# castorini/dhr

Measured on AMD Instinct MI355X. Metric: queries/sec (exact top-1000, brute-force dense-hybrid GIP retrieval), higher is better.
Workload: dtype i8 (bound GEMM: gated AND ungated columns int8 x int8 -> int32 on the matrix cores, every gated rounding upward, the ungated quantisation error paid by the filter margin) + f64-accumulated f16 x f32 exact rescoring of the survivors -- the returned scores are the exact scores rounded once, identical

## Files before the change

### dhr_amd/csrc/kernels.hip

```cpp
#include <algorithm>
#include <cstdlib>
#include <mutex>

#include "dhr_internal.h"
#include "gemm_common.h"
#include <type_traits>

namespace dhr {

typedef short short8 __attribute__((ext_vector_type(8)));

static hipError_t ensure_lds_attr(const void* fn, int bytes, int (&have)[64]) {
  static std::mutex mu;
  int dev = 0;
  (void)hipGetDevice(&dev);
  std::lock_guard<std::mutex> lock(mu);
  if (bytes <= have[dev & 63]) return hipSuccess;
  const hipError_t e = hipFuncSetAttribute(fn, hipFuncAttributeMaxDynamicSharedMemorySize, bytes);
  if (e == hipSuccess) have[dev & 63] = bytes;
  return e;
}

__device__ __forceinline__ float wave_sum(float v) {
#pragma unroll
// ... 1117 lines not shown
#pragma unroll
      for (int u = 0; u < U; ++u) {
        if constexpr (PB == 8) { const uint2 t = gather8(r + u * 128); v[u].w[0] = t.x; v[u].w[1] = t.y; }
        else { const uint4 t = gather16(r + u * 128); v[u].w[0] = t.x; v[u].w[1] = t.y; v[u].w[WPP - 2] = t.z; v[u].w[WPP - 1] = t.w; }
      }
    }
  };
  uint2 c;
  Piece v[U];
  fetch(base + (threadIdx.x / LPC), c, v);
  for (uint32_t i = base + (threadIdx.x / LPC); i < base + REFINE_PER_WG; i += CPR) {
    uint2 cn;
    Piece vn[U];
    fetch(i + CPR < base + REFINE_PER_WG ? i + CPR : 0xffffffffu, cn, vn);
    int isum = 0;
#pragma unroll
    for (int u = 0; u < U; ++u) {
#pragma unroll
      for (int h = 0; h < WPP; ++h) {
        isum = __builtin_amdgcn_sdot4((int)fe[WPP * u + h], (int)(v[u].w[h] & 0x0f0f0f0fu), isum, false);
        isum = __builtin_amdgcn_sdot4((int)fo[WPP * u + h], (int)((v[u].w[h] >> 4) & 0x0f0f0f0fu), isum, false);
      }
    }
#pragma unroll
    for (int o = 1; o < LPC; o <<= 1) isum += __shfl_xor(isum, o, 64);
    if (sub == 0 && i < count) {
      float u2 = __uint_as_float(c.y) + sa * (float)(isum - off);
      u2 += fabsf(u2) * 4.8e-7f;
      if (u2 >= t) {
        const uint32_t slot = atomicAdd(p.out_cnt + q, 1u);
        if (slot < p.out_cap) p.out[(int64_t)q * p.out_cap + slot] = make_uint2(c.x, __float_as_uint(u2));
      }
    }
    c = cn;
#pragma unroll
    for (int u = 0; u < U; ++u) v[u] = vn[u];
  }
  if (!p.blk_off) return;
  }
}
hipError_t launch_refine(const RefineArgs& a, hipStream_t s) {
  if (a.max_count == 0 || a.n_queries <= 0) return hipSuccess;
  if (a.resid8) {
    const dim3 grid = a.blk_off ? dim3(std::min<uint32_t>(a.flat_blocks, FLAT_GRID_MAX)) : dim3((a.max_count + REFINE_PER_WG - 1) / REFINE_PER_WG, (unsigned)a.n_queries);
    if (a.blk_off && !a.flat_blocks) return hipSuccess;
    switch (a.resid_ld / 8) {
      case 16: hipLaunchKernelGGL(dense_refine_kernel<16>, grid, dim3(256), 0, s, a); break;
      case 32: hipLaunchKernelGGL(dense_refine_kernel<32>, grid, dim3(256), 0, s, a); break;
      case 48: hipLaunchKernelGGL(dense_refine_kernel<48>, grid, dim3(256), 0, s, a); break;
      case 64: hipLaunchKernelGGL(dense_refine_kernel<64>, grid, dim3(256), 0, s, a); break;
      default: return hipErrorInvalidValue;
    }
    return hipGetLastError();
  }
  const bool g8 = a.g8_q8 != nullptr;
  const size_t lds = (size_t)a.d_dlr * (g8 ? 8 : 4);
  const dim3 grid = a.blk_off ? dim3(std::min<uint32_t>(a.flat_blocks, FLAT_GRID_MAX)) : dim3((a.max_count + REFINE_PER_WG - 1) / REFINE_PER_WG, (unsigned)a.n_queries);
  if (a.blk_off && !a.flat_blocks) return hipSuccess;
  if (g8) hipLaunchKernelGGL(refine_kernel<true>, grid, dim3(256), lds, s, a);
  else hipLaunchKernelGGL(refine_kernel<false>, grid, dim3(256), lds, s, a);
  return hipGetLastError();
}

__device__ __forceinline__ float fmix_lo(uint32_t a, uint32_t b) { float r; asm("v_fma_mix_f32 %0, %1, %2, 0 op_sel_hi:[1,1,0]" : "=v"(r) : "v"(a), "v"(b)); return r; }
__device__ __forceinline__ float fmix_hi(uint32_t a, uint32_t b) { float r; asm("v_fma_mix_f32 %0, %1, %2, 0 op_sel:[1,1,0] op_sel_hi:[1,1,0]" : "=v"(r) : "v"(a), "v"(b)); return r; }
typedef unsigned short ushort2v __attribute__((ext_vector_type(2)));
__device__ __forceinline__ uint32_t pair_mask(uint32_t x, uint32_t sel) {
  union { uint32_t u; ushort2v v; } t, one;
  t.u = __builtin_amdgcn_perm(0u, x, sel);
  one.u = 0x00010001u;
  t.v = __builtin_elementwise_min(t.v, one.v);
  t.v = t.v - one.v;
  return t.u;
}
__device__ __forceinline__ uint32_t pair_mask16(uint32_t x) {
  union { uint32_t u; ushort2v v; } t, one;
  t.u = x;
  one.u = 0x00010001u;
  t.v = __builtin_elementwise_min(t.v, one.v);
  t.v = t.v - one.v;
  return t.u;
}
template <int PATH>
__device__ __forceinline__ void rescore_block(const RescoreArgs& p, const int q, const uint32_t blk) {
  const int lane = threadIdx.x & 63;
  const int wave = threadIdx.x >> 6;
  uint32_t count;
  if (p.cand) { count = p.cnt[q]; if (count > p.cap) count = p.cap; }
  else if (p.rows32) count = p.count_all;
  else count = p.count_all;
  const uint32_t base = blk * RESCORE_CANDS_PER_WG;
  if (base >= count) return;
  const float* q32 = p.q32 + (int64_t)q * p.k_rm;
  const int16_t* qi = p.q_idx + (int64_t)q * p.d_dlr;
  const int nchunks = p.k_rm >> 3;
  const int dlr_chunks = p.d_dlr >> 3;
  const bool fast = p.q16 && *p.q_inexact == 0u && (!p.gate || p.d_dlr == 0 || p.c_idx_dtype == DHR_IDX_U8 || p.c_idx_dtype == DHR_IDX_I8);
  const bool some_zero = p.q_inexact && p.q_inexact[1] != 0u;
  uint32_t nz_mask = some_zero ? 0u : 0xFFFFFFFFu;
  for (int c = lane, t = 0; some_zero && c < nchunks; c += 64, ++t) {
    const float4 qa = *(const float4*)(q32 + c * 8);
    const float4 qb = *(const float4*)(q32 + c * 8 + 4);
    if (qa.x != 0.f || qa.y != 0.f || qa.z != 0.f || qa.w != 0.f || qb.x != 0.f || qb.y != 0.f || qb.z != 0.f || qb.w != 0.f) nz_mask |= 1u << t;
  }
  if constexpr (PATH == 0) {
    if (p.split && p.q16 && *p.q_inexact == 0u && some_zero) {
      int m = 0;
      for (int t = 0; t * 64 < nchunks; ++t) m += __popcll(__ballot((nz_mask >> t) & 1u));
      if (m <= 16) return;
    }
  }
  if constexpr (PATH == 3) {
    if (!(p.q16 && *p.q_inexact == 0u && some_zero)) return;
    const bool idx16 = p.c_idx_dtype == DHR_IDX_I16;
    int nzc[16];
    int m = 0;
    for (int c0 = 0, t = 0; c0 < nchunks && m <= 16; c0 += 64, ++t) {
      uint64_t b = __ballot((nz_mask >> t) & 1u);
      while (b && m <= 16) { if (m < 16) nzc[m] = c0 + (__ffsll((unsigned long long)b) - 1); ++m; b &= b - 1; }
    }
    if (m > 16) return;
    {
      auto run = [&](auto lanes_c) __attribute__((always_inline)) {
        constexpr int L = decltype(lanes_c)::value, P = 64 / L;
        const int ci = lane / L, sl = lane % L;
        int myc = -1;
#pragma unroll
        for (int e = 0; e < L; ++e) if (e < m && sl == e) myc = nzc[e];
        uint4 qv = make_uint4(0u, 0u, 0u, 0u);
        uint4 qix = make_uint4(0u, 0u, 0u, 0u);
        const bool gated_chunk = myc >= 0 && myc < dlr_chunks && p.gate;
        if (myc >= 0) qv = *(const uint4*)(p.q16 + (int64_t)q * p.k_rm + myc * 8);
        if (gated_chunk) {
          if (idx16) qix = *(const uint4*)(p.q_idx + (int64_t)q * p.d_dlr + myc * 8);
          else { const uint2 t8 = *(const uint2*)(p.q_idx8 + (int64_t)q * p.d_dlr + myc * 8); qix.x = t8.x; qix.y = t8.y; }
        }
        static_assert(RESCORE_CANDS_PER_WG % (4 * P) == 0, "4 waves x P pairs per round");
        for (uint32_t i0 = base + wave * P; i0 < base + RESCORE_CANDS_PER_WG && i0 < count; i0 += 4 * P) {
          const uint32_t i = i0 + ci;
          const bool live = i < count;
          uint32_t row = 0u;
          if (live) {
            if (p.cand) row = p.cand[(int64_t)q * p.cap + i].x;
            else if (p.rows32) row = p.rows32[(int64_t)q * p.ld_rows + i];
            else row = (uint32_t)(p.row0 + i);
          }
          const bool valid = live && (int64_t)row < p.n_rows;
          double acc = 0.0;
          if (valid && myc >= 0) {
            const uint4 dv = *(const uint4*)(p.vals_rm + (int64_t)row * p.k_rm + myc * 8);
            uint32_t d[4] = {dv.x, dv.y, dv.z, dv.w};
            const uint32_t qq[4] = {qv.x, qv.y, qv.z, qv.w};
            if (gated_chunk && idx16) {
              const uint4 cix = *(const uint4*)((const int16_t*)p.c_idx + (int64_t)row * p.d_dlr + myc * 8);
              d[0] &= pair_mask16(cix.x ^ qix.x); d[1] &= pair_mask16(cix.y ^ qix.y);
              d[2] &= pair_mask16(cix.z ^ qix.z); d[3] &= pair_mask16(cix.w ^ qix.w);
            } else if (gated_chunk) {
              const uint2 cix = *(const uint2*)((const uint8_t*)p.c_idx + (int64_t)row * p.d_dlr + myc * 8);
              const uint32_t x0 = cix.x ^ qix.x, x1 = cix.y ^ qix.y;
              d[0] &= pair_mask(x0, 0x0c010c00u); d[1] &= pair_mask(x0, 0x0c030c02u);
              d[2] &= pair_mask(x1, 0x0c010c00u); d[3] &= pair_mask(x1, 0x0c030c02u);
            }
#pragma unroll
            for (int e = 0; e < 4; ++e) {
              acc += (double)fmix_lo(d[e], qq[e]);
              acc += (double)fmix_hi(d[e], qq[e]);
            }
          }
#pragma unroll
          for (int o = 1; o < L; o <<= 1) acc += __shfl_xor(acc, o, 64);
          if (sl == 0 && live) {
            const float sc = valid ? (float)acc : -INFINITY;
            if (p.out_keys) p.out_keys[(int64_t)q * p.ld_keys + i] = valid ? make_key(sc, row) : 0ull;
            if (p.out_scores && q < p.n_queries) p.out_scores[(int64_t)q * p.ld_scores + i] = sc;
          }
        }
      };
      if (m <= 8) run(std::integral_constant<int, 8>{}); else run(std::integral_constant<int, 16>{});
      return;
    }
  }
  if constexpr (PATH != 3) {
  if constexpr (PATH == 0 || PATH == 2)
  if (fast && !some_zero && nchunks <= 128) {
#ifndef RESCORE_NARROW_L
#define RESCORE_NARROW_L 16
#endif
    constexpr int L = RESCORE_NARROW_L, P = 64 / L;
    const int g = lane / L, sl = lane % L;
    static_assert(RESCORE_CANDS_PER_WG % (4 * P) == 0, "4 waves x P pairs per round");
    for (uint32_t i0 = base + wave * P; i0 < base + RESCORE_CANDS_PER_WG && i0 < count; i0 += 4 * P) {
      const uint32_t i = i0 + g;
      const bool live = i < count;
      uint32_t row = 0u;
      if (live) {
        if (p.cand) row = p.cand[(int64_t)q * p.cap + i].x;
        else if (p.rows32) row = p.rows32[(int64_t)q * p.ld_rows + i];
        else row = (uint32_t)(p.row0 + i);
      }
      const bool valid = live && (int64_t)row < p.n_rows;
      double acc = 0.0;
      if (valid) {
        for (int c = sl; c < nchunks; c += L) {
          const uint4 dv = gather16(p.vals_rm + (int64_t)row * p.k_rm + c * 8);
          const uint4 qv = *(const uint4*)(p.q16 + (int64_t)q * p.k_rm + c * 8);
          uint32_t d[4] = {dv.x, dv.y, dv.z, dv.w};
          const uint32_t qq[4] = {qv.x, qv.y, qv.z, qv.w};
          if (c < dlr_chunks && p.gate) {
            const uint2 ci = gather8((const uint8_t*)p.c_idx + (int64_t)row * p.d_dlr + c * 8);
            const uint2 qi8 = *(const uint2*)(p.q_idx8 + (int64_t)q * p.d_dlr + c * 8);
            const uint32_t x0 = ci.x ^ qi8.x, x1 = ci.y ^ qi8.y;
            d[0] &= pair_mask(x0, 0x0c010c00u); d[1] &= pair_mask(x0, 0x0c030c02u);
            d[2] &= pair_mask(x1, 0x0c010c00u); d[3] &= pair_mask(x1, 0x0c030c02u);
          }
#pragma unroll
          for (int e = 0; e < 4; ++e) {
            acc += (double)fmix_lo(d[e], qq[e]);
            acc += (double)fmix_hi(d[e], qq[e]);
          }
        }
      }
#pragma unroll
      for (int o = L / 2; o > 0; o >>= 1) acc += __shfl_xor(acc, o, 64);
      if (sl == 0 && live) {
        const float sc = valid ? (float)acc : -INFINITY;
        if (p.out_keys) p.out_keys[(int64_t)q * p.ld_keys + i] = valid ? make_key(sc, row) : 0ull;
        if (p.out_scores && q < p.n_queries) p.out_scores[(int64_t)q * p.ld_scores + i] = sc;
      }
    }
    return;
  }
  if constexpr (PATH != 2)
  for (uint32_t i = base + wave; i < base + RESCORE_CANDS_PER_WG && i < count; i += 4) {
    uint32_t row;
    if (p.cand) row = p.cand[(int64_t)q * p.cap + i].x;
    else if (p.rows32) row = p.rows32[(int64_t)q * p.ld_rows + i];
    else row = (uint32_t)(p.row0 + i);
    const bool valid = (int64_t)row < p.n_rows;
    double acc = 0.0;
    if (valid && fast) {
      for (int c = lane; c < nchunks; c += 64) {
        if (!((nz_mask >> (c >> 6)) & 1u)) continue;
        const uint4 dv = gather16(p.vals_rm + (int64_t)row * p.k_rm + c * 8);
        const uint4 qv = *(const uint4*)(p.q16 + (int64_t)q * p.k_rm + c * 8);
        uint32_t d[4] = {dv.x, dv.y, dv.z, dv.w};
        const uint32_t qq[4] = {qv.x, qv.y, qv.z, qv.w};
        if (c < dlr_chunks && p.gate) {
          const uint2 ci = gather8((const uint8_t*)p.c_idx + (int64_t)row * p.d_dlr + c * 8);
          const uint2 qi8 = *(const uint2*)(p.q_idx8 + (int64_t)q * p.d_dlr + c * 8);
          const uint32_t x0 = ci.x ^ qi8.x, x1 = ci.y ^ qi8.y;
          d[0] &= pair_mask(x0, 0x0c010c00u); d[1] &= pair_mask(x0, 0x0c030c02u);
          d[2] &= pair_mask(x1, 0x0c010c00u); d[3] &= pair_mask(x1, 0x0c030c02u);
        }
#pragma unroll
        for (int e = 0; e < 4; ++e) {
          acc += (double)fmix_lo(d[e], qq[e]);
          acc += (double)fmix_hi(d[e], qq[e]);
        }
      }
      acc = wave_sum_f64(acc);
    } else if (PATH == 0 && valid) {
      for (int c = lane; c < nchunks; c += 64) {
        if (!((nz_mask >> (c >> 6)) & 1u)) continue;
        const half8 dv = *(const half8*)(p.vals_rm + (int64_t)row * p.k_rm + c * 8);
        const float4 qa = *(const float4*)(q32 + c * 8);
        const float4 qb = *(const float4*)(q32 + c * 8 + 4);
        const float qv[8] = {qa.x, qa.y, qa.z, qa.w, qb.x, qb.y, qb.z, qb.w};
        if (c < dlr_chunks && p.gate) {
          int ci[8];
          if (p.c_idx_dtype == DHR_IDX_I16) {
            const short8 v = *(const short8*)((const int16_t*)p.c_idx + (int64_t)row * p.d_dlr + c * 8);
#pragma unroll
            for (int e = 0; e < 8; ++e) ci[e] = v[e];
          } else {
            const uint2 v = *(const uint2*)((const uint8_t*)p.c_idx + (int64_t)row * p.d_dlr + c * 8);
#pragma unroll
            for (int e = 0; e < 8; ++e) {
              const uint32_t w = (e < 4) ? v.x : v.y;
              const uint32_t byte = (w >> (8 * (e & 3))) & 0xFFu;
              ci[e] = (p.c_idx_dtype == DHR_IDX_I8) ? (int)(int8_t)byte : (int)byte;
            }
          }
          const short8 qiv = *(const short8*)(qi + c * 8);
#pragma unroll
          for (int e = 0; e < 8; ++e) {
            const double d = (ci[e] == (int)qiv[e]) ? (double)(float)dv[e] : 0.0;
            acc = fma(d, (double)qv[e], acc);
          }
        } else {
#pragma unroll
          for (int e = 0; e < 8; ++e) acc = fma((double)(float)dv[e], (double)qv[e], acc);
        }
      }
      acc = wave_sum_f64(acc);
    }
    if (lane == 0) {
      const float sc = valid ? (float)acc : -INFINITY;
      if (p.out_keys) p.out_keys[(int64_t)q * p.ld_keys + i] = valid ? make_key(sc, row) : 0ull;
      if (p.out_scores && q < p.n_queries) p.out_scores[(int64_t)q * p.ld_scores + i] = sc;
    }
  }
  }
}
#ifndef RESCORE_WPE
#define RESCORE_WPE 7
#endif
__device__ __forceinline__ bool rescore_fast_batch(const RescoreArgs& p) {
  return p.q16 && p.q_inexact[0] == 0u && p.q_inexact[1] == 0u &&
         (!p.gate || p.d_dlr == 0 || p.c_idx_dtype == DHR_IDX_U8 || p.c_idx_dtype == DHR_IDX_I8);
}
template <int PATH>
__device__ __forceinline__ void rescore_run(const RescoreArgs& p) {
  if (!p.blk_off) { rescore_block<PATH>(p, (int)blockIdx.y, blockIdx.x); return; }
  for (uint32_t b = blockIdx.x;; b += gridDim.x) {
    int q; uint32_t blk;
    if (!flat_block(p.blk_off, p.n_queries, b, q, blk)) return;
    rescore_block<PATH>(p, q, blk);
  }
}
__global__ void __launch_bounds__(256) __attribute__((amdgpu_waves_per_eu(RESCORE_WPE))) rescore_kernel(RescoreArgs p) {
  if (p.split && rescore_fast_batch(p)) return;
  rescore_run<0>(p);
}
__global__ void __launch_bounds__(256) __attribute__((amdgpu_waves_per_eu(8))) rescore_fast_kernel(RescoreArgs p) {
  if (!rescore_fast_batch(p) || (p.k_rm >> 3) <= 128) return;
  rescore_run<1>(p);
}
__global__ void __launch_bounds__(256) __attribute__((amdgpu_waves_per_eu(8))) rescore_sparse_kernel(RescoreArgs p) {
  if (!p.q16 || p.q_inexact[0] != 0u || p.q_inexact[1] == 0u) return;
  rescore_run<3>(p);
}
__global__ void __launch_bounds__(256) __attribute__((amdgpu_waves_per_eu(8))) rescore_narrow_kernel(RescoreArgs p) {
  if (!rescore_fast_batch(p) || (p.k_rm >> 3) > 128) return;
  rescore_run<2>(p);
}
hipError_t launch_rescore(const RescoreArgs& a_in, hipStream_t s) {
  if (a_in.max_count == 0 || a_in.n_queries <= 0) return hipSuccess;
  RescoreArgs a = a_in;
  a.split = (a.q16 && a.q_inexact) ? 1 : 0;
  const bool wide = (a.k_rm >> 3) > 128;
  dim3 grid;
  if (a.blk_off) {
    if (!a.flat_blocks) return hipSuccess;
    grid = dim3(std::min<uint32_t>(a.flat_blocks, FLAT_GRID_MAX));
  } else grid = dim3((a.max_count + RESCORE_CANDS_PER_WG - 1) / RESCORE_CANDS_PER_WG, (unsigned)a.n_queries);
  if (a.split && wide) hipLaunchKernelGGL(rescore_fast_kernel, grid, dim3(256), 0, s, a);
  if (a.split && !wide) hipLaunchKernelGGL(rescore_narrow_kernel, grid, dim3(256), 0, s, a);
  if (a.split) hipLaunchKernelGGL(rescore_sparse_kernel, grid, dim3(256), 0, s, a);
  hipLaunchKernelGGL(rescore_kernel, grid, dim3(256), 0, s, a);
  return hipGetLastError();
}

__device__ __forceinline__ void bitonic_desc(uint64_t* keys, int n, int tid, int nthreads) {
  for (int size = 2; size <= n; size <<= 1) {
    for (int stride = size >> 1; stride > 0; stride >>= 1) {
      for (int t = tid; t < (n >> 1); t += nthreads) {
        const int pos = 2 * t - (t & (stride - 1));
        const uint64_t a = keys[pos], b = keys[pos + stride];
        const bool desc = (pos & size) == 0;
        if ((a < b) == desc) { keys[pos] = b; keys[pos + stride] = a; }
      }
      __syncthreads();
    }
  }
}

__device__ __forceinline__ int count_greater(const uint64_t* arr, int n, uint64_t key) {
  int lo = 0, hi = n;
  while (lo < hi) {
    const int mid = (lo + hi) >> 1;
    if (arr[mid] > key) lo = mid + 1; else hi = mid;
  }
  return lo;
}

constexpr int SELECT_SM_THREADS = 256;
template <int EA>
__global__ void __launch_bounds__(SELECT_SM_THREADS) select_kernel(SelectArgs p) {
  extern __shared__ __attribute__((aligned(16))) char smem[];
  uint64_t* A = (uint64_t*)smem;
  int& fill = *(int*)(smem + (size_t)p.sort_n * 8);
  const int kps = p.kps;
  uint64_t* B = A + kps;
  const int q = blockIdx.x;
  const int tid = threadIdx.x;
  uint32_t count = p.cnt ? p.cnt[q] : p.count_all;
  if (p.cnt && count > p.cap) count = p.cap;
  uint64_t* topk = p.topk_keys + (int64_t)q * p.kp;
  const uint64_t* in = p.in_keys + (int64_t)q * p.ld_keys;
  for (int j = tid; j < kps; j += SELECT_SM_THREADS) A[j] = topk[j];
  if (tid == 0) fill = 0;
  __syncthreads();
  uint32_t room = 64;
  while (room * 2 <= (uint32_t)(p.sort_n - kps) && room < 2048) room <<= 1;
  const int k_keep = p.k_keep ? p.k_keep : p.k;
  for (uint32_t base = 0; base < count; base += room) {
    const uint64_t kth = A[k_keep - 1];
    __syncthreads();
    const uint32_t end = (base + room < count) ? base + room : count;
    for (uint32_t j = base + tid; j < end; j += SELECT_SM_THREADS) {
      const uint64_t key = in[j];
      if (key > kth) B[atomicAdd(&fill, 1)] = key;
    }
    __syncthreads();
    const int m = fill;
    if (m > 0) {
      int m2 = 2;
      while (m2 < m) m2 <<= 1;
      for (int j = m + tid; j < m2; j += SELECT_SM_THREADS) B[j] = 0ull;
      __syncthreads();
      bitonic_desc(B, m2, tid, SELECT_SM_THREADS);
      uint64_t ka[EA], kb[8];
      int da[EA], db[8];
#pragma unroll
      for (int e = 0; e < EA; ++e) {
        const int i = tid + e * SELECT_SM_THREADS;
        da[e] = kps;
        if (i < kps) { ka[e] = A[i]; da[e] = ka[e] ? i + count_greater(B, m, ka[e]) : kps; }
      }
#pragma unroll
      for (int e = 0; e < 8; ++e) {
        const int j = tid + e * SELECT_SM_THREADS;
        db[e] = kps;
        if (j < m) { kb[e] = B[j]; db[e] = j + count_greater(A, kps, kb[e]); }
      }
      const int total = min(kps, m + count_greater(A, kps, 0ull));
      __syncthreads();
      for (int j = total + tid; j < kps; j += SELECT_SM_THREADS) A[j] = 0ull;
#pragma unroll
      for (int e = 0; e < EA; ++e)
        if (da[e] < kps) A[da[e]] = ka[e];
#pragma unroll
      for (int e = 0; e < 8; ++e)
        if (db[e] < kps) A[db[e]] = kb[e];
    }
    __syncthreads();
    if (tid == 0) fill = 0;
    __syncthreads();
  }
  for (int j = tid; j < kps; j += SELECT_SM_THREADS) topk[j] = (j < k_keep) ? A[j] : 0ull;
  if (tid == 0) {
    const uint64_t kth = A[p.k - 1];
    float t = kth ? ordered_f32((uint32_t)(kth >> 32)) : -INFINITY;
    if (p.monotone) t = fmaxf(t, p.tau[q]);
    p.tau[q] = t;
    p.thr[q] = (q < p.n_queries) ? t - p.margin[q] : INFINITY;
  }
}

constexpr int SELECT_BIG_BATCH = 2048;
constexpr int SELECT_BIG_THREADS = 256;
constexpr int SELECT_BIG_EPT = 4;
__global__ void __launch_bounds__(SELECT_BIG_THREADS) select_big_kernel(SelectArgs p) {
  __shared__ uint64_t B[SELECT_BIG_BATCH];
  __shared__ int fill;
  const int q = blockIdx.x, tid = threadIdx.x;
  uint32_t count = p.cnt ? p.cnt[q] : p.count_all;
  if (p.cnt && count > p.cap) count = p.cap;
  uint64_t* topk = p.topk_keys + (int64_t)q * p.kp;
  const uint64_t* in = p.in_keys + (int64_t)q * p.ld_keys;
  const int k_keep = p.k_keep ? p.k_keep : p.k;
  constexpr int TILE = SELECT_BIG_THREADS * SELECT_BIG_EPT;
  for (uint32_t base = 0; base < count; base += SELECT_BIG_BATCH) {
    if (tid == 0) fill = 0;
    __syncthreads();
    const uint64_t kth = topk[k_keep - 1];
    const uint32_t end = (base + SELECT_BIG_BATCH < count) ? base + SELECT_BIG_BATCH : count;
    for (uint32_t j = base + tid; j < end; j += SELECT_BIG_THREADS) {
      const uint64_t key = in[j];
      if (key > kth) B[atomicAdd(&fill, 1)] = key;
    }
    __syncthreads();
    const int m = fill;
    if (m == 0) continue;
    int m2 = 2;
    while (m2 < m) m2 <<= 1;
    for (int j = m + tid; j < m2; j += SELECT_BIG_THREADS) B[j] = 0ull;
    __syncthreads();
    bitonic_desc(B, m2, tid, SELECT_BIG_THREADS);
    uint64_t kb[SELECT_BIG_BATCH / SELECT_BIG_THREADS]; int db[SELECT_BIG_BATCH / SELECT_BIG_THREADS];
#pragma unroll
    for (int e = 0; e < SELECT_BIG_BATCH / SELECT_BIG_THREADS; ++e) {
      const int j = tid + e * SELECT_BIG_THREADS;
      kb[e] = (j < m) ? B[j] : 0ull;
      db[e] = (j < m) ? j + count_greater(topk, k_keep, kb[e]) : k_keep;
    }
    __syncthreads();
    for (int t0 = (k_keep - 1) / TILE * TILE; t0 >= 0; t0 -= TILE) {
      uint64_t ka[SELECT_BIG_EPT]; int da[SELECT_BIG_EPT];
#pragma unroll
      for (int e = 0; e < SELECT_BIG_EPT; ++e) {
        const int i = t0 + tid + e * SELECT_BIG_THREADS;
        da[e] = k_keep;
        if (i < k_keep) { ka[e] = topk[i]; da[e] = i + count_greater(B, m, ka[e]); }
      }
      __syncthreads();
#pragma unroll
      for (int e = 0; e < SELECT_BIG_EPT; ++e)
        if (da[e] < k_keep) topk[da[e]] = ka[e];
    }
#pragma unroll
    for (int e = 0; e < SELECT_BIG_BATCH / SELECT_BIG_THREADS; ++e)
      if (db[e] < k_keep) topk[db[e]] = kb[e];
  }
  __syncthreads();
  if (tid == 0) {
    const uint64_t kth = topk[p.k - 1];
    float t = kth ? ordered_f32((uint32_t)(kth >> 32)) : -INFINITY;
    if (p.monotone) t = fmaxf(t, p.tau[q]);
    p.tau[q] = t;
    p.thr[q] = (q < p.n_queries) ? t - p.margin[q] : INFINITY;
  }
}

hipError_t launch_select(const SelectArgs& a, hipStream_t s) {
  if (a.kp > 16384) return launch_select_global(a, s);
  if (a.kp > 4096) {
    hipLaunchKernelGGL(select_big_kernel, dim3((unsigned)a.n_queries), dim3(SELECT_BIG_THREADS), 0, s, a);
    return hipGetLastError();
  }
  static int attr_bytes[64] = {}, attr_bytes4[64] = {};
  const int bytes = a.sort_n * 8 + 16;
  if (a.kp <= 4 * SELECT_SM_THREADS) {
    if (hipError_t e = ensure_lds_attr((const void*)select_kernel<4>, bytes, attr_bytes4); e != hipSuccess) return e;
    hipLaunchKernelGGL(select_kernel<4>, dim3((unsigned)a.n_queries), dim3(SELECT_SM_THREADS), bytes, s, a);
    return hipGetLastError();
  }
  if (hipError_t e = ensure_lds_attr((const void*)select_kernel<16>, bytes, attr_bytes); e != hipSuccess) return e;
  hipLaunchKernelGGL(select_kernel<16>, dim3((unsigned)a.n_queries), dim3(SELECT_SM_THREADS), bytes, s, a);
  return hipGetLastError();
}

constexpr int PQ_K = 256;
constexpr int PQ_MAX_DSUB = 64;

template <int DSUB>
__global__ void __launch_bounds__(256) pq_assign_kernel(const __half* __restrict__ vals, int64_t ld, int64_t n, int64_t stride, int dsub_rt,
                                                        const float* __restrict__ cb , uint8_t* __restrict__ codes,
                                                        int64_t ld_codes, float* __restrict__ sums ,
                                                        uint32_t* __restrict__ counts , float* __restrict__ err ,
                                                        int ksub ) {
  __shared__ float c[PQ_K * PQ_MAX_DSUB];
  __shared__ float cn[PQ_K];
  const int dsub = DSUB ? DSUB : dsub_rt;
  const int m = blockIdx.y;
  const float* cbm = cb + (int64_t)m * ksub * dsub;
  for (int i = threadIdx.x; i < ksub * dsub; i += 256) c[i] = cbm[i];
  __syncthreads();
  if ((int)threadIdx.x < ksub) {
    float s = 0.f;
    for (int j = 0; j < dsub; ++j) s += c[threadIdx.x * dsub + j] * c[threadIdx.x * dsub + j];
    cn[threadIdx.x] = s;
  }
  __syncthreads();
  const int64_t pi = (int64_t)blockIdx.x * 256 + threadIdx.x;
  if (pi >= n) return;
  const __half* x = vals + pi * stride * ld + (int64_t)m * dsub;
  float xv[DSUB ? DSUB : PQ_MAX_DSUB];
#pragma unroll
  for (int j = 0; j < (DSUB ? DSUB : PQ_MAX_DSUB); ++j)
    if (j < dsub) xv[j] = __half2float(x[j]);
  float best = INFINITY;
  int arg = 0;
  for (int k = 0; k < ksub; ++k) {
    float dot = 0.f;
#pragma unroll
    for (int j = 0; j < (DSUB ? DSUB : 1); ++j)
      if (DSUB) dot += xv[j] * c[k * dsub + j];
    if (!DSUB)
      for (int j = 0; j < dsub; ++j) dot += xv[j] * c[k * dsub + j];
    const float dist = cn[k] - 2.f * dot;
    if (dist < best) { best = dist; arg = k; }
  }
  if (codes) codes[pi * ld_codes + m] = (uint8_t)arg;
  if (sums) {
    for (int j = 0; j < dsub; ++j) atomicAdd(&sums[((int64_t)m * ksub + arg) * dsub + j], xv[j]);
    atomicAdd(&counts[m * ksub + arg], 1u);
    if (err) {
      float xx = 0.f;
      for (int j = 0; j < dsub; ++j) xx += xv[j] * xv[j];
      atomicAdd(&err[m], best + xx);
    }
  }
}
__global__ void __launch_bounds__(256) pq_update_kernel(float* __restrict__ cb, const float* __restrict__ sums, const uint32_t* __restrict__ counts,
                                                        int dsub, int ksub) {
  const int m = blockIdx.x, k = threadIdx.x;
  __shared__ uint32_t cnt[PQ_K];
  __shared__ int big;
  cnt[k] = k < ksub ? counts[m * ksub + k] : 0u;
  __syncthreads();
  if (k == 0) {
    int b = 0;
    for (int i = 1; i < ksub; ++i) if (cnt[i] > cnt[b]) b = i;
    big = b;
  }
  __syncthreads();
  if (k >= ksub) return;
  float* c = cb + ((int64_t)m * ksub + k) * dsub;
  if (cnt[k] > 0) {
    const float inv = 1.f / (float)cnt[k];
    for (int j = 0; j < dsub; ++j) c[j] = sums[((int64_t)m * ksub + k) * dsub + j] * inv;
  } else {
    const float inv = 1.f / (float)(cnt[big] ? cnt[big] : 1u);
    for (int j = 0; j < dsub; ++j) c[j] = sums[((int64_t)m * ksub + big) * dsub + j] * inv * (1.f + ((j + k) & 1 ? 1.f : -1.f) / 1024.f);
  }
}
__global__ void __launch_bounds__(256) pq_init_kernel(const __half* __restrict__ vals, int64_t ld, int64_t n, int64_t stride, int dsub, int M,
                                                      float* __restrict__ cb, int ksub) {
  const int m = blockIdx.x, k = threadIdx.x;
  if (k >= ksub) return;
  const int64_t pi = (n >= ksub) ? (int64_t)k * (n / ksub) : (int64_t)(k % (n > 0 ? n : 1));
  const __half* x = vals + pi * stride * ld + (int64_t)m * dsub;
  for (int j = 0; j < dsub; ++j) cb[((int64_t)m * ksub + k) * dsub + j] = __half2float(x[j]);
}
__global__ void __launch_bounds__(256) pq_decode_kernel(const uint8_t* __restrict__ codes, int64_t ld_codes, int64_t n, int M, int dsub,
                                                        const float* __restrict__ cb, __half* __restrict__ out, int64_t ld_out, int ksub) {
  const int d = M * dsub;
  const int64_t total = n * d;
  for (int64_t g = (int64_t)blockIdx.x * 256 + threadIdx.x; g < total; g += (int64_t)gridDim.x * 256) {
    const int64_t row = g / d;
    const int col = (int)(g - row * d);
    const int m = col / dsub, j = col - m * dsub;
    out[row * ld_out + col] = __float2half(cb[((int64_t)m * ksub + codes[row * ld_codes + m]) * dsub + j]);
  }
}
hipError_t launch_pq_init(const __half* vals, int64_t ld, int64_t n, int64_t stride, int dsub, int M, float* cb, int ksub, hipStream_t s) {
  hipLaunchKernelGGL(pq_init_kernel, dim3(M), dim3(256), 0, s, vals, ld, n, stride, dsub, M, cb, ksub);
  return hipGetLastError();
}
hipError_t launch_pq_assign(const __half* vals, int64_t ld, int64_t n, int64_t stride, int dsub, int M, const float* cb, uint8_t* codes,
                            int64_t ld_codes, float* sums, uint32_t* counts, float* err, int ksub, hipStream_t s) {
  if (n <= 0) return hipSuccess;
  const dim3 grid((unsigned)((n + 255) / 256), M);
#define PQ_GO(D) hipLaunchKernelGGL(pq_assign_kernel<D>, grid, dim3(256), 0, s, vals, ld, n, stride, dsub, cb, codes, ld_codes, sums, counts, err, ksub)
  if (dsub == 12) PQ_GO(12); else if (dsub == 24) PQ_GO(24); else if (dsub == 14) PQ_GO(14); else if (dsub == 16) PQ_GO(16); else PQ_GO(0);
#undef PQ_GO
  return hipGetLastError();
}
hipError_t launch_pq_update(float* cb, const float* sums, const uint32_t* counts, int dsub, int M, int ksub, hipStream_t s) {
  hipLaunchKernelGGL(pq_update_kernel, dim3(M), dim3(256), 0, s, cb, sums, counts, dsub, ksub);
  return hipGetLastError();
}
hipError_t launch_pq_decode(const uint8_t* codes, int64_t ld_codes, int64_t n, int M, int dsub, const float* cb, __half* out, int64_t ld_out, int ksub,
                            hipStream_t s) {
  if (n <= 0) return hipSuccess;
  const int64_t blocks = std::min<int64_t>((n * M * dsub + 255) / 256, 65536);
  hipLaunchKernelGGL(pq_decode_kernel, dim3((unsigned)blocks), dim3(256), 0, s, codes, ld_codes, n, M, dsub, cb, out, ld_out, ksub);
  return hipGetLastError();
// ... 463 lines not shown
```

Measured before the change: 60370.

## Add templated wide rescore kernel with in-flight row prefetch and register-resident query

Adds a specialised rescore kernel for wide rows, templated on the number of 64-lane chunks (T) and gated index chunks (G). It keeps the query slice in registers, double-buffers candidate row gathers (P rows in flight) so loads overlap the f64 accumulation, and replaces the shuffle reduction with ds_swizzle. Gating masks are computed with packed u16 min/sub. Per-(T,G) waves-per-EU choices are meant to trade occupancy against the register cost of holding several rows in flight, and unsupported shapes fall back to the old kernel.

```diff
diff --git a/dhr_amd/csrc/kernels.hip b/dhr_amd/csrc/kernels.hip
--- a/dhr_amd/csrc/kernels.hip
+++ b/dhr_amd/csrc/kernels.hip
@@ -1443,6 +1443,138 @@
   }
   }
 }
+__device__ __forceinline__ double wave_sum_f64_swz(double v) {
+  v += __shfl_xor(v, 32, 64);
+  auto step = [&](auto o) __attribute__((always_inline)) {
+    constexpr int pat = (decltype(o)::value << 10) | 0x1F;
+    union { double d; int w[2]; } a, b;
+    a.d = v;
+    b.w[0] = __builtin_amdgcn_ds_swizzle(a.w[0], pat);
+    b.w[1] = __builtin_amdgcn_ds_swizzle(a.w[1], pat);
+    v += b.d;
+  };
+  step(std::integral_constant<int, 16>{}); step(std::integral_constant<int, 8>{}); step(std::integral_constant<int, 4>{});
+  step(std::integral_constant<int, 2>{}); step(std::integral_constant<int, 1>{});
+  return v;
+}
+__device__ __forceinline__ uint32_t pair_mask_pk(uint32_t x, uint32_t sel, uint32_t one) {
+  uint32_t t = __builtin_amdgcn_perm(0u, x, sel), r;
+  asm("v_pk_min_u16 %0, %1, %2" : "=v"(r) : "v"(t), "v"(one));
+  asm("v_pk_sub_u16 %0, %1, %2" : "=v"(t) : "v"(r), "v"(one));
+  return t;
+}
+#ifndef RESCORE_WIDE_P
+#define RESCORE_WIDE_P 2
+#endif
+constexpr int rescore_wide_wpe(int T, int G) {
+#ifdef RESCORE_WIDE_WPE
+  return RESCORE_WIDE_WPE;
+#else
+  static_assert(RESCORE_WIDE_P == 2, "the table below was taken from the P = 2 allocation");
+  return T == 3 ? (G <= 2 ? 7 : 6) : (G == 0 ? 7 : G <= 3 ? 5 : 4);
+#endif
+}
+template <int T, int G, int P>
+__device__ __forceinline__ void rescore_block_wide(const RescoreArgs& p, const int q_in, const uint32_t blk_in) {
+  constexpr int NP = RESCORE_CANDS_PER_WG / 4;
+  static_assert(NP <= 64 && G <= T && P >= 1, "one lane per pair of the wave");
+  const int lane = threadIdx.x & 63;
+  const int wave = __builtin_amdgcn_readfirstlane(threadIdx.x >> 6);
+  const int q = __builtin_amdgcn_readfirstlane(q_in);
+  const uint32_t blk = (uint32_t)__builtin_amdgcn_readfirstlane((int)blk_in);
+  uint32_t count;
+  if (p.cand) { count = p.cnt[q]; if (count > p.cap) count = p.cap; }
+  else count = p.count_all;
+  count = (uint32_t)__builtin_amdgcn_readfirstlane((int)count);
+  const uint32_t first = blk * RESCORE_CANDS_PER_WG + wave;
+  if (first >= count) return;
+  const int npairs = (int)min((uint32_t)NP, (count - first + 3u) >> 2);
+  const uint32_t nchunks = (uint32_t)p.k_rm >> 3;
+  const uint32_t dlr_chunks = (uint32_t)p.d_dlr >> 3;
+  const uint32_t i_own = first + 4u * (uint32_t)lane;
+  uint32_t row_own = 0u;
+  bool valid_own = false;
+  if (lane < npairs) {
+    if (p.cand) row_own = p.cand[(int64_t)q * p.cap + i_own].x;
+    else if (p.rows32) row_own = p.rows32[(int64_t)q * p.ld_rows + i_own];
+    else row_own = (uint32_t)(p.row0 + i_own);
+    valid_own = (int64_t)row_own < p.n_rows;
+  }
+  const uint32_t row_ld = valid_own ? row_own : 0u;
+  const uint32_t c_last = (uint32_t)lane + 64u * (T - 1);
+  const bool live_last = c_last < nchunks;
+  const uint32_t voff0 = (uint32_t)lane * 16u, voff_last = (live_last ? c_last : nchunks - 1u) * 16u;
+  const uint32_t g_last = (uint32_t)lane + 64u * (G > 0 ? G - 1 : 0);
+  const bool gated_last = g_last < dlr_chunks;
+  const uint32_t xoff0 = (uint32_t)lane * 8u, xoff_last = (gated_last ? g_last : dlr_chunks - 1u) * 8u;
+  const uint32_t gmask_last = gated_last ? 0xFFFFFFFFu : 0u;
+  uint4 qv[T];
+  uint2 qx[G > 0 ? G : 1];
+  {
+    const char* q16 = (const char*)(p.q16 + (int64_t)q * p.k_rm);
+#pragma unroll
+    for (int t = 0; t < T; ++t) qv[t] = *(const uint4*)(q16 + (t < T - 1 ? voff0 + 1024u * t : voff_last));
+    if constexpr (G > 0) {
+      const char* q8 = (const char*)(p.q_idx8 + (int64_t)q * p.d_dlr);
+#pragma unroll
+      for (int t = 0; t < G; ++t) qx[t] = *(const uint2*)(q8 + (t < G - 1 ? xoff0 + 512u * t : xoff_last));
+    }
+  }
+  uint4 dv[P][T];
+  uint2 dx[P][G > 0 ? G : 1];
+  auto issue = [&](const int s, const uint32_t row) __attribute__((always_inline)) {
+    uint32_t v0 = voff0, v1 = voff_last, x0 = xoff0, x1 = xoff_last;
+    asm volatile("" : "+v"(v0), "+v"(v1), "+v"(x0), "+v"(x1));
+    const char* r = (const char*)(p.vals_rm + (int64_t)row * p.k_rm);
+#pragma unroll
+    for (int t = 0; t < T; ++t) dv[s][t] = gather16(r + (t < T - 1 ? v0 + 1024u * t : v1));
+    if constexpr (G > 0) {
+      const char* x = (const char*)p.c_idx + (int64_t)row * p.d_dlr;
+#pragma unroll
+      for (int t = 0; t < G; ++t) dx[s][t] = gather8(x + (t < G - 1 ? x0 + 512u * t : x1));
+    }
+  };
+  const uint32_t one = 0x00010001u;
+  auto chunk = [&](double acc, const int s, const int t) __attribute__((always_inline)) -> double {
+    uint32_t d[4] = {dv[s][t].x, dv[s][t].y, dv[s][t].z, dv[s][t].w};
+    const uint32_t qq[4] = {qv[t].x, qv[t].y, qv[t].z, qv[t].w};
+    if (t < G) {
+      uint32_t x0 = dx[s][t].x ^ qx[t].x, x1 = dx[s][t].y ^ qx[t].y;
+      if (t == G - 1) { x0 &= gmask_last; x1 &= gmask_last; }
+      d[0] &= pair_mask_pk(x0, 0x0c010c00u, one); d[1] &= pair_mask_pk(x0, 0x0c030c02u, one);
+      d[2] &= pair_mask_pk(x1, 0x0c010c00u, one); d[3] &= pair_mask_pk(x1, 0x0c030c02u, one);
+    }
+#pragma unroll
+    for (int e = 0; e < 4; ++e) {
+      acc += (double)fmix_lo(d[e], qq[e]);
+      acc += (double)fmix_hi(d[e], qq[e]);
+    }
+    return acc;
+  };
+#pragma unroll
+  for (int j = 0; j < P && j < NP; ++j) issue(j, (uint32_t)__builtin_amdgcn_readlane((int)row_ld, j));
+#pragma unroll
+  for (int t = 0; t < T; ++t) asm volatile("" : "+v"(qv[t].x), "+v"(qv[t].y), "+v"(qv[t].z), "+v"(qv[t].w));
+  float res = 0.f;
+#pragma unroll
+  for (int j = 0; j < NP; ++j) {
+    if (j >= npairs) break;
+    const int s = j % P;
+    double acc = 0.0;
+#pragma unroll
+    for (int t = 0; t < T - 1; ++t) acc = chunk(acc, s, t);
+    if (live_last) acc = chunk(acc, s, T - 1);
+    __builtin_amdgcn_sched_barrier(0);
+    if (j + P < NP) issue(s, (uint32_t)__builtin_amdgcn_readlane((int)row_ld, j + P));
+    acc = wave_sum_f64_swz(acc);
+    if (lane == j) res = (float)acc;
+  }
+  if (lane < npairs) {
+    const float sc = valid_own ? res : -INFINITY;
+    if (p.out_keys) p.out_keys[(int64_t)q * p.ld_keys + i_own] = valid_own ? make_key(sc, row_own) : 0ull;
+    if (p.out_scores && q < p.n_queries) p.out_scores[(int64_t)q * p.ld_scores + i_own] = sc;
+  }
+}
 #ifndef RESCORE_WPE
 #define RESCORE_WPE 7
 #endif
@@ -1450,14 +1582,18 @@
   return p.q16 && p.q_inexact[0] == 0u && p.q_inexact[1] == 0u &&
          (!p.gate || p.d_dlr == 0 || p.c_idx_dtype == DHR_IDX_U8 || p.c_idx_dtype == DHR_IDX_I8);
 }
-template <int PATH>
-__device__ __forceinline__ void rescore_run(const RescoreArgs& p) {
-  if (!p.blk_off) { rescore_block<PATH>(p, (int)blockIdx.y, blockIdx.x); return; }
+template <class F>
+__device__ __forceinline__ void rescore_for_blocks(const RescoreArgs& p, F block) {
+  if (!p.blk_off) { block((int)blockIdx.y, blockIdx.x); return; }
   for (uint32_t b = blockIdx.x;; b += gridDim.x) {
     int q; uint32_t blk;
     if (!flat_block(p.blk_off, p.n_queries, b, q, blk)) return;
-    rescore_block<PATH>(p, q, blk);
-  }
+    block(q, blk);
+  }
+}
+template <int PATH>
+__device__ __forceinline__ void rescore_run(const RescoreArgs& p) {
+  rescore_for_blocks(p, [&](const int q, const uint32_t blk) __attribute__((always_inline)) { rescore_block<PATH>(p, q, blk); });
 }
 __global__ void __launch_bounds__(256) __attribute__((amdgpu_waves_per_eu(RESCORE_WPE))) rescore_kernel(RescoreArgs p) {
   if (p.split && rescore_fast_batch(p)) return;
@@ -1466,6 +1602,11 @@
 __global__ void __launch_bounds__(256) __attribute__((amdgpu_waves_per_eu(8))) rescore_fast_kernel(RescoreArgs p) {
   if (!rescore_fast_batch(p) || (p.k_rm >> 3) <= 128) return;
   rescore_run<1>(p);
+}
+template <int T, int G>
+__global__ void __launch_bounds__(256) __attribute__((amdgpu_waves_per_eu(rescore_wide_wpe(T, G)))) rescore_fast_kernel_wide(RescoreArgs p) {
+  if (!rescore_fast_batch(p)) return;
+  rescore_for_blocks(p, [&](const int q, const uint32_t blk) __attribute__((always_inline)) { rescore_block_wide<T, G, RESCORE_WIDE_P>(p, q, blk); });
 }
 __global__ void __launch_bounds__(256) __attribute__((amdgpu_waves_per_eu(8))) rescore_sparse_kernel(RescoreArgs p) {
   if (!p.q16 || p.q_inexact[0] != 0u || p.q_inexact[1] == 0u) return;
@@ -1485,7 +1626,18 @@
     if (!a.flat_blocks) return hipSuccess;
     grid = dim3(std::min<uint32_t>(a.flat_blocks, FLAT_GRID_MAX));
   } else grid = dim3((a.max_count + RESCORE_CANDS_PER_WG - 1) / RESCORE_CANDS_PER_WG, (unsigned)a.n_queries);
-  if (a.split && wide) hipLaunchKernelGGL(rescore_fast_kernel, grid, dim3(256), 0, s, a);
+  if (a.split && wide) {
+    const int nch = a.k_rm >> 3, T = (nch + 63) / 64;
+    const int G = (a.gate && a.d_dlr > 0) ? ((a.d_dlr >> 3) + 63) / 64 : 0;
+    const bool inflight = (T == 3 || T == 4) && G <= T && (a.k_rm & 7) == 0 && (a.d_dlr & 7) == 0 && a.n_rows > 0;
+    switch (inflight ? T * 8 + G : 0) {
+#define DHR_RESCORE_WIDE(T_, G_) case T_ * 8 + G_: hipLaunchKernelGGL((rescore_fast_kernel_wide<T_, G_>), grid, dim3(256), 0, s, a); break;
+      DHR_RESCORE_WIDE(3, 0) DHR_RESCORE_WIDE(3, 1) DHR_RESCORE_WIDE(3, 2) DHR_RESCORE_WIDE(3, 3)
+      DHR_RESCORE_WIDE(4, 0) DHR_RESCORE_WIDE(4, 1) DHR_RESCORE_WIDE(4, 2) DHR_RESCORE_WIDE(4, 3) DHR_RESCORE_WIDE(4, 4)
+#undef DHR_RESCORE_WIDE
+      default: hipLaunchKernelGGL(rescore_fast_kernel, grid, dim3(256), 0, s, a);
+    }
+  }
   if (a.split && !wide) hipLaunchKernelGGL(rescore_narrow_kernel, grid, dim3(256), 0, s, a);
   if (a.split) hipLaunchKernelGGL(rescore_sparse_kernel, grid, dim3(256), 0, s, a);
   hipLaunchKernelGGL(rescore_kernel, grid, dim3(256), 0, s, a);
```

After: 61840 (median of 6 runs). 2.4% higher.
